# alibaba/nann

Measured on AMD Instinct MI355X. Metric: retrieval QPS @ recall@200 parity, 1M items/128-d, higher is better.
Workload: dtype f16 rows / f32 L2

## Files before the change

nann_amd/csrc/nann_device.h:

```cpp
#pragma once
#include <type_traits>
#include <hip/hip_runtime.h>
#include <hip/hip_fp16.h>
#include <stdint.h>

namespace nann {

constexpr int kNT = 1024;
constexpr int kNW = kNT / 64;
constexpr int kTopkEPT = 16;
constexpr int kMaxK = 1024;
constexpr int kPhaseScratch = 27648;
constexpr int kMaxD = 512;
constexpr int kLdsScoresOff = 10752;
constexpr int kLdsScores = 4096;

enum : int { DT_F16 = 0, DT_BF16 = 1, DT_F32 = 2 };

__device__ __forceinline__ int local_tid() {
  int t = threadIdx.x;
  asm volatile("" : "+v"(t));
  __builtin_assume(t >= 0 && t < 1024);
  return t;
}
// ... 457 lines not shown
  }
  __syncthreads();
  int base = 0;
  for (int c = 0; c < n_chunks; ++c) {
    const bool more = c + 1 < n_chunks;
    if (more) issue(c + 1, first_row(c + 1) + wave, B);
    const int n_c = min(kChunk, G - c * kChunk);
    long long tw = pt.now();
    base = wg_filter_chunk<kLdsBm, NT>(S, n_c, bm, n_items, out, base);
    pt.sub(PH_EX_WALKBUSY, tw);
    if (more) {
      commit(c + 1, B);
      rest(c + 1, B.r0);
    }
    __syncthreads();
  }
  pt.sub(PH_EX_LOOP, tsub);
  const int bad = S->bad;
  __syncthreads();
  return bad ? -1 : base;
}

constexpr uint32_t kVisEmpty = 0xffffffffu;
constexpr int kVisPosBits = 12;
constexpr int kVisStepBits = 6;
template <int NT, int SLOTS>
struct ExpandHashScratch {
  static constexpr int PER = 4096 / NT;
  static constexpr int kMaskBits = 2 * SLOTS;
  static constexpr int kMaskWords = kMaskBits / 32;
  uint32_t rowdelta[kMaxK];
  uint32_t startmask[kMaskWords];
  unsigned short maskprefix[kMaskWords];
  unsigned long long kept[64];
  uint32_t wave_tot[2 * kNW];
  int flags[4];
};

constexpr int kVisTagBits = 14;
constexpr int kVisMinPiece = 512;
constexpr int kVisDirectBits = 32 - kVisPosBits;
template <int SLOTS, bool TAG>
__device__ __forceinline__ void vis_key(int32_t x, int id_bits, uint32_t& h0, uint32_t& hi) {
  static_assert(SLOTS == 16384 || SLOTS == 32768, "14 or 15 hash bits");
  constexpr int HB = SLOTS == 16384 ? 14 : 15;
  if constexpr (!TAG) {
// ... 42 lines not shown
        const uint32_t c = atomicCAS(&vis[h], kVisEmpty, val);
        if (c == kVisEmpty) break;
        if ((c ^ val) < kStepOne) { S->flags[1] = 1; break; }
        if (step_inc && (val & kStepEnd) == kStepEnd) { S->flags[2] = 1; break; }
        h = (h + step) & (SLOTS - 1);
        val += step_inc;
      }
      out[i] = id;
    } else {
      S->flags[0] = 1;
    }
  }
  __syncthreads();
  const int bad = S->flags[0], dup = S->flags[1], far = S->flags[2];
  __syncthreads();
  return bad ? -1 : far ? -2 : dup ? -4 : n;
}

template <int NT, int SLOTS, bool TAG>
__device__ __forceinline__ int wg_expand_hash_impl(const int32_t* frontier, int n_frontier,
                                              const int32_t* __restrict__ values,
                                              const int64_t* __restrict__ row_splits, uint32_t n_items,
                                              uint32_t* vis, int id_bits, int& vis_count, int32_t* out,
                                              unsigned char* scratch, int* gathered, SubTimer pt) {
  using Scratch = ExpandHashScratch<NT, SLOTS>;
  constexpr int PER = Scratch::PER;
  constexpr int NWV = NT / 64;
  static_assert(PER * NWV == 64, "one keep-mask word per lane");
  Scratch* S = reinterpret_cast<Scratch*>(scratch);
  long long tsub = pt.now();
  const int tid = local_tid(), lane = tid & 63;
  const int wave = __builtin_amdgcn_readfirstlane(tid >> 6);
  const uint64_t lt = lanemask_lt(lane);
  const bool list_mode = row_splits == nullptr;
  const int n_rows = list_mode ? 1 : n_frontier;
  if (tid < 4) S->flags[tid] = 0;
  for (int i = tid; i < Scratch::kMaskWords; i += NT) S->startmask[i] = 0u;
  __syncthreads();
  uint32_t total = 0, rows_ne = 0;
  for (int t0 = 0; t0 < n_rows; t0 += NT) {
    const int t = t0 + tid;
    uint32_t len = 0, start = 0;
    if (list_mode) {
      if (t == 0) len = (uint32_t)n_frontier;
    } else if (t < n_frontier) {
      const int32_t node = frontier[t];
      if ((uint32_t)node < n_items) {
        const int64_t s = row_splits[node], e = row_splits[node + 1];
        start = (uint32_t)s;
        len = (uint32_t)(e - s);
      } else {
        S->flags[0] = 1;
      }
    }
    const uint32_t ne = len ? 1u : 0u;
    const uint32_t inc = wave_scan_add(len), inc_ne = wave_scan_add(ne);
    if (lane == 63) { S->wave_tot[wave] = inc; S->wave_tot[kNW + wave] = inc_ne; }
    __syncthreads();
    uint32_t wbase = 0, tot = 0, wbase_ne = 0, tot_ne = 0;
#pragma unroll
    for (int w = 0; w < NWV; ++w) {
      const uint32_t v = S->wave_tot[w], vn = S->wave_tot[kNW + w];
      if (w < wave) { wbase += v; wbase_ne += vn; }
      tot += v; tot_ne += vn;
    }
    const uint32_t my_off = total + wbase + inc - len;
    if (len && my_off < (uint32_t)Scratch::kMaskBits) {
// ... 133 lines not shown
    vis_count += tot;
    if (cut) {
      if (c_next < G) fetch(c_next, min(PL, G - c_next), x);
    } else {
#pragma unroll
      for (int j = 0; j < PER; ++j) x[j] = xn[j];
    }
    c0 = c_next;
    pt.sub(PH_EX_RANK, tw);
  }
  pt.sub(PH_EX_LOOP, tsub);
  if (__ballot(bad) != 0ull && lane == 0) S->flags[0] = 1;
  __syncthreads();
  const int any_bad = S->flags[0];
  __syncthreads();
  return any_bad ? -1 : base;
}

template <int NT, int SLOTS>
__device__ __forceinline__ int wg_expand_hash(const int32_t* frontier, int n_frontier,
                                              const int32_t* __restrict__ values,
                                              const int64_t* __restrict__ row_splits, uint32_t n_items,
                                              uint32_t* vis, int id_bits, int& vis_count, int32_t* out,
                                              unsigned char* scratch, int* gathered, SubTimer pt) {
  if (id_bits <= kVisDirectBits)
    return wg_expand_hash_impl<NT, SLOTS, false>(frontier, n_frontier, values, row_splits, n_items, vis, id_bits,
                                                 vis_count, out, scratch, gathered, pt);
  return wg_expand_hash_impl<NT, SLOTS, true>(frontier, n_frontier, values, row_splits, n_items, vis, id_bits,
                                              vis_count, out, scratch, gathered, pt);
}

template <int DT>
struct RowChunk {
  uint4 a;
  uint4 b;
};

template <int DT>
__device__ __forceinline__ RowChunk<DT> load_chunk(const void* table, size_t row, int d, int sub) {
  RowChunk<DT> r;
  if constexpr (DT == DT_F32) {
    const uint4* p = reinterpret_cast<const uint4*>(static_cast<const float*>(table) + row * d + sub * 8);
    r.a = p[0];
    r.b = p[1];
  } else {
    const uint4* p = reinterpret_cast<const uint4*>(static_cast<const uint16_t*>(table) + row * d + sub * 8);
    r.a = p[0];
    r.b = make_uint4(0, 0, 0, 0);
  }
  return r;
}

// ... 193 lines not shown

template <int KCAP>
struct TopkScratchT {
  unsigned long long sel[KCAP < 512 ? 512 : KCAP];
  union {
    unsigned short prank[kNT];
    struct { uint32_t above[256]; uint32_t cursor[256]; } bins;
  };
  uint32_t misc[4];
  uint32_t wlo[kNW], whi[kNW];
  uint32_t wcnt[kNW];
};
static_assert(kNT * sizeof(unsigned short) == 512 * sizeof(uint32_t), "the bin tables overlay the partial ranks");
typedef TopkScratchT<kMaxK> TopkScratch;
static_assert(sizeof(TopkScratch) <= kLdsScoresOff, "top-k scratch overlaps the LDS scores");
static_assert(kLdsScoresOff + kLdsScores * 4 <= kPhaseScratch, "phase scratch too small");
static_assert(sizeof(ExpandWalkScratch) <= kPhaseScratch, "phase scratch too small");

template <int NS, bool SCL, int NT, int KCAP = kMaxK, bool BIN = false>
__device__ __forceinline__ int wg_topk_impl(const int32_t* ids, const float* scores,
                                            const float* lds_scores, int n, int k, int32_t* out_pos,
                                            int32_t* out_ids, float* out_scores, const int64_t* id_map,
                                            int64_t* out_mapped, unsigned char* scratch, SubTimer pt,
                                            int n_all = 0x7fffffff, uint32_t floor_key = 0u) {
  TopkScratchT<KCAP>* S = reinterpret_cast<TopkScratchT<KCAP>*>(scratch);
  long long tsub = pt.now();
  const int tid = local_tid(), lane = tid & 63, wave = tid >> 6;
  const uint64_t lt = lanemask_lt(lane);
  constexpr bool REG = NS > 0;
  uint32_t key[REG ? NS : 1];
  if constexpr (REG) {
    float raw[NS];
#pragma unroll
    for (int j = 0; j < NS; ++j) {
      const int i = min(j * NT + tid, n - 1);
      raw[j] = SCL ? lds_scores[i] : scores[i];
    }
#pragma unroll
    for (int j = 0; j < NS; ++j) key[j] = (j * NT + tid < n) ? score_key(raw[j]) : 0u;
  }
#define NANN_FOR_KEYS(...)                                                    \
  if constexpr (REG) {                                                        \
    _Pragma("unroll") for (int j = 0; j < NS; ++j) {                          \
      const int i = j * NT + tid;                                             \
      const uint32_t kj = key[j];                                             \
      const bool valid = i < n && (!BIN || i < n_all || kj > floor_key);      \
      __VA_ARGS__                                                             \
// ... 153 lines not shown
      const uint64_t m = __ballot(e);
      if (lane == 0) S->wcnt[wave] = (uint32_t)popc64(m);
      __syncthreads();
      uint32_t wb = 0, tot = 0;
      for (int w = 0; w < NT / 64; ++w) {
        const uint32_t t = S->wcnt[w];
        if (w < wave) wb += t;
        tot += t;
      }
      const uint32_t rank = eq_base + wb + (uint32_t)popc64(m & lt);
      if (e && rank < r) S->sel[c_gt + rank] = ((unsigned long long)kj << 32) | (uint32_t)(~(uint32_t)i);
      eq_base += tot;
      __syncthreads();
    })
  }
#undef NANN_FOR_KEYS
  __syncthreads();
  pt.sub(PH_TK_COLLECT, tsub);
  int K2 = 64;
  while (K2 < k) K2 <<= 1;
  const bool split = K2 <= NT;
  int32_t my_id = 0;
  if (tid < k && ids) my_id = ids[(int)(~(uint32_t)(S->sel[tid] & 0xffffffffull))];
  const bool binned = use_bins && S->misc[3] == 0u;
  if (split && !binned) {
    const int segs = NT / K2;
    const int e = tid & (K2 - 1), seg = tid / K2;
    const int len = (k + segs - 1) / segs;
    const int o0 = seg * len, o1 = min(k, o0 + len);
    int pr = 0;
    if (e < k) {
      const unsigned long long mine = S->sel[e];
      int o = o0;
      for (; o + 8 <= o1; o += 8) {
        unsigned long long v[8];
#pragma unroll
        for (int u = 0; u < 8; ++u) v[u] = S->sel[o + u];
#pragma unroll
        for (int u = 0; u < 8; ++u) pr += (v[u] > mine) ? 1 : 0;
      }
      for (; o < o1; ++o) pr += (S->sel[o] > mine) ? 1 : 0;
    }
    S->prank[tid] = (unsigned short)pr;
    __syncthreads();
  }
  for (int e = tid; e < k; e += NT) {
// ... 15 lines not shown
    } else if (split) {
      for (int sg = 0; sg < NT / K2; ++sg) rank += S->prank[sg * K2 + e];
    } else {
      int o = 0;
      for (; o + 8 <= k; o += 8) {
        unsigned long long v[8];
#pragma unroll
        for (int u = 0; u < 8; ++u) v[u] = S->sel[o + u];
#pragma unroll
        for (int u = 0; u < 8; ++u) rank += (v[u] > mine) ? 1 : 0;
      }
      for (; o < k; ++o) rank += (S->sel[o] > mine) ? 1 : 0;
    }
    const int pos = (int)(~(uint32_t)(mine & 0xffffffffull));
    const int32_t idv = ids ? (e == tid ? my_id : ids[pos]) : pos;
    if (out_pos) out_pos[rank] = pos;
    if (out_ids) out_ids[rank] = idv;
    if (out_scores) {
      const uint32_t kbits = (uint32_t)(mine >> 32);
      const uint32_t u = (kbits & 0x80000000u) ? (kbits & 0x7fffffffu) : ~kbits;
      out_scores[rank] = (u != 0u) ? __uint_as_float(u) : (SCL ? lds_scores[pos] : scores[pos]);
    }
    if (out_mapped) out_mapped[rank] = id_map[idv];
  }
  __syncthreads();
  pt.sub(PH_TK_SORT, tsub);
  return 0;
}

template <int NT = kNT, int KCAP = kMaxK, bool BIN = false>
__device__ __forceinline__ int wg_topk(const int32_t* ids, const float* scores, const float* lds_scores,
                                       int n, int k, int32_t* out_pos, int32_t* out_ids,
                                       float* out_scores, const int64_t* id_map, int64_t* out_mapped,
                                       unsigned char* scratch, SubTimer pt = no_timer()) {
  if (k < 0 || k > KCAP) return 7;
  if (n < k) return 4;
  if (k == 0) return 0;
#define NANN_TOPK_CASE(NS_, SCL_)                                                                   \
  return wg_topk_impl<NS_, SCL_, NT, KCAP, BIN>(ids, scores, lds_scores, n, k, out_pos, out_ids, out_scores, \
                                           id_map, out_mapped, scratch, pt)
  if (lds_scores != nullptr && n <= kLdsScores) {
    if (n <= 1 * NT) NANN_TOPK_CASE(1, true);
    if (n <= 2 * NT) NANN_TOPK_CASE(2, true);
    if (n <= 4 * NT) NANN_TOPK_CASE(4, true);
    if constexpr (8 * NT <= kLdsScores) NANN_TOPK_CASE(8, true);
  }
  if (n <= 1 * NT) NANN_TOPK_CASE(1, false);
  if (n <= 2 * NT) NANN_TOPK_CASE(2, false);
  if (n <= 4 * NT) NANN_TOPK_CASE(4, false);
  if (n <= 8 * NT) NANN_TOPK_CASE(8, false);
  if (n <= kTopkEPT * NT) NANN_TOPK_CASE(kTopkEPT, false);
  NANN_TOPK_CASE(0, false);
#undef NANN_TOPK_CASE
}

template <int NT, int KCAP>
__device__ __forceinline__ int wg_topk_binned(const int32_t* ids, const float* scores, int n, int k, int32_t* out_ids,
                                              float* out_scores, unsigned char* scratch, int n_all = 0x7fffffff,
                                              uint32_t floor_key = 0u) {
  if (k < 0 || k > KCAP) return 7;
  if (n < k) return 4;
  if (k == 0) return 0;
  if (n <= 4 * NT) return wg_topk_impl<4, false, NT, KCAP, true>(ids, scores, nullptr, n, k, nullptr, out_ids, out_scores, nullptr, nullptr, scratch, no_timer(), n_all, floor_key);
// ... 6 lines not shown
```

nann_amd/csrc/nann_hip.hip:

```cpp
#include "nann_eval.h"
#include "nann_attn.h"
#include "nann_order_kernels.h"
#include "nann_scan.h"
#include "host/nann_graphdef_text.h"
#include "host/nann_blaze_options.h"
#include "host/nann_npy.h"
#include "host/nann_projcache.h"

#include <algorithm>
#include <atomic>
#include <cmath>
#include <cstddef>
#include <cstdio>
#include <cstdlib>
#include <cstring>
#include <fstream>
#include <limits>
#include <memory>
#include <mutex>
#include <string>
#include <vector>

#include <sys/stat.h>

// ... 603 lines not shown
    if (hipMemGetInfo(free_b, &total) == hipSuccess) return true;
    (void)hipGetLastError();
    return false;
  }
  static bool event_create(Event* e) {
    if (hipEventCreateWithFlags(e, hipEventDisableTiming) == hipSuccess) return true;
    (void)hipGetLastError();
    return false;
  }
  static void event_destroy(Event e) { (void)hipEventDestroy(e); }
  static void event_record(Event e, Stream s) { (void)hipEventRecord(e, s); }
  static bool event_done(Event e) { return hipEventQuery(e) != hipErrorNotReady; }
  static void event_wait(Event e) { (void)hipEventSynchronize(e); }
};
typedef nann::ProjCacheT<HipProjBackend> ProjCache;
typedef nann::ProjTableT<HipProjBackend> ProjTable;
struct SearchOpt {
  int mode;
  int reserve;
  int preproject;
  int mlp_form;
  int small32;
  int order;
};
static std::atomic<int> g_traversal_mode{-1}, g_slot_reserve{-1}, g_preproject{-1};
static const SearchOpt& env_defaults() {
  static const SearchOpt d = [] {
    SearchOpt o{NANN_TRAVERSAL_AUTO, 0, 1, NANN_MLP_FORM_AUTO, 1, 1};
    if (const char* e = std::getenv("NANN_PREPROJECT")) o.preproject = !(e[0] == '0' && e[1] == 0);
    if (const char* e = std::getenv("NANN_SEARCH_SLOT_RESERVE")) o.reserve = std::max(0, std::atoi(e));
    if (const char* e = std::getenv("NANN_MLP_FORM")) o.mlp_form = std::string(e) == "fused" ? NANN_MLP_FORM_FUSED : std::string(e) == "phased" ? NANN_MLP_FORM_PHASED : NANN_MLP_FORM_AUTO;
    if (const char* e = std::getenv("NANN_PHASE_SMALL32")) o.small32 = !(e[0] == '0');
    if (const char* e = std::getenv("NANN_QUERY_ORDER")) o.order = !(e[0] == '0');
    return o;
  }();
  return d;
}
static SearchOpt resolve_options(const nann_search_options* u) {
  SearchOpt o = env_defaults();
  const int gm = g_traversal_mode.load(std::memory_order_relaxed), gr = g_slot_reserve.load(std::memory_order_relaxed),
            gp = g_preproject.load(std::memory_order_relaxed);
  if (gm >= 0) o.mode = gm;
  if (gr >= 0) o.reserve = gr;
  if (gp >= 0) o.preproject = gp;
  if (u) {
    const size_t nb = u->struct_bytes > 0 ? (size_t)u->struct_bytes : sizeof(*u);
    auto has = [&](const int32_t* f) { return (size_t)(reinterpret_cast<const char*>(f) - reinterpret_cast<const char*>(u)) + 4 <= nb; };
    if (has(&u->traversal_mode) && u->traversal_mode >= 0) o.mode = u->traversal_mode;
    if (has(&u->slot_reserve) && u->slot_reserve >= 0) o.reserve = u->slot_reserve;
    if (has(&u->preprojection) && u->preprojection >= 0) o.preproject = u->preprojection != 0;
    if (has(&u->mlp_form) && u->mlp_form >= 0) o.mlp_form = u->mlp_form;
  }
  return o;
}
static int check_options(const nann_search_options* u) {
  if (!u) return NANN_OK;
// ... 1195 lines not shown
                            : kind < 0 ? big_scratch : (size_t)kPhaseScratch;
  const bool bitmap_fits = !res && bm_bytes + bm_scratch + tail <= di.lds_max;
  const int mode = opt.mode;
  const int bm_vis = (bitmap_fits && mode != NANN_TRAVERSAL_HBM_BITMAP) ? VIS_LDS_BITMAP : VIS_HBM_BITMAP;
  const size_t bm_lds = bm_scratch + tail + (bm_vis == VIS_LDS_BITMAP ? bm_bytes : 0);
  const int bm_per_cu = (bm_vis == VIS_LDS_BITMAP || res) ? 1 : 2;
  const int id_bits = std::max(16, bit_length((uint64_t)std::max<int64_t>(ix->desc.n_items, 1)));
  const bool tag_fits = id_bits <= 27;
  const double mean_deg0 = (double)ix->desc.nb_nnz[0] / (double)std::max<int64_t>(ix->desc.n_items, 1);
  const double walk_deg = std::min<double>((double)ix->max_deg[0], 2.75 * mean_deg0);
  const double rows_walked = (double)t[1] + t[2] + t[3];
  const double est_guess = t[1] + 0.45 * walk_deg * rows_walked;
  const double est_visited = ix->probe_valid ? std::min(t[1] + std::min(1.15 * (double)ix->probe_new_per_row_q90, (double)ix->probe_new_per_row_max) * rows_walked,
                                                        t[1] + (double)ix->max_deg[0] * rows_walked)
                                             : est_guess;
  const bool tag_entries = id_bits > 20;
  const double fit16 = !ix->probe_valid ? 11000.0 : tag_entries ? 13000.0 : 15000.0;
  const double fit32 = !ix->probe_valid ? 24000.0 : tag_entries ? 26000.0 : 30500.0;
  const double worst_visited = t[1] + (double)ix->max_deg[0] * ((double)t[1] + t[2] + t[3]);
  const size_t hash16_lds = (size_t)vis_slots(VIS_LDS_HASH) * 4 + hash_phase_scratch<512, 16384>() + tail;
  const size_t hash32_lds = (size_t)vis_slots(VIS_LDS_HASH32) * 4 + hash_phase_scratch<kNT, 32768>() + tail;
  const bool hash_ok = (kind == NANN_SCORER_L2 || kind < 0) && tag_fits && 2 * hash16_lds <= di.lds_max &&
                       hash32_lds <= di.lds_max;
  int hash_vis = -1;
  if (mode == NANN_TRAVERSAL_LDS_HASH) hash_vis = VIS_LDS_HASH;
  else if (mode == NANN_TRAVERSAL_LDS_HASH32) hash_vis = VIS_LDS_HASH32;
  else if (mode == NANN_TRAVERSAL_AUTO && (kind == NANN_SCORER_L2 || kind < 0)) {
    if (worst_visited <= 16320.0 || est_visited <= fit16) hash_vis = VIS_LDS_HASH;
    else if (worst_visited <= 32704.0 || est_visited <= fit32) hash_vis = VIS_LDS_HASH32;
    if (hash_vis == VIS_LDS_HASH && kind == NANN_SCORER_L2 && n_queries <= (int64_t)di.cus) hash_vis = VIS_LDS_HASH32;
  }
  const bool fits16 = worst_visited <= 16320.0 || est_visited <= fit16 || mode == NANN_TRAVERSAL_LDS_HASH;
  const bool own_hash_plan = (kind == kKindAttn || kind == kKindMlpSplit || res) && tag_fits && fits16;
  if ((mode == NANN_TRAVERSAL_LDS_HASH || mode == NANN_TRAVERSAL_LDS_HASH32) && !hash_ok && kind >= 0 &&
      !(own_hash_plan && mode == NANN_TRAVERSAL_LDS_HASH))
    return fail(NANN_ERR_UNSUPPORTED, "hash-set traversal: shards below 2^27 items; the 32K-slot set: L2 scorer only");
  unsigned long long off[9];
  uint32_t gbm_words = bm_vis == VIS_HBM_BITMAP ? ix->bm_words : 0u;
  if (res || kind < 0 || kind == kKindAttn) gbm_words = std::max<uint32_t>(std::max<uint32_t>(gbm_words, ix->bm_words), (uint32_t)vis_slots(kind < 0 ? VIS_LDS_HASH32 : VIS_LDS_HASH));
  p->slot_bytes = slot_layout(p->max_cand, p->max_raw, p->pool_cap, gbm_words, off);
  p->id_bits = id_bits;
  p->fb_vis = bm_vis;
  p->fb_lds_bytes = bm_lds;
  p->fb_slots = (int)std::max<int64_t>(1, std::min<int64_t>(n_queries, (int64_t)di.cus * bm_per_cu));
  if (own_hash_plan && mode != NANN_TRAVERSAL_LDS_BITMAP && mode != NANN_TRAVERSAL_HBM_BITMAP) {
    p->vis = VIS_LDS_HASH;
    p->nt = 512;
    p->lds_bytes = res ? (size_t)kMlpResBytes + hash_phase_scratch<512, 16384>() + tail
                       : (size_t)vis_slots(VIS_LDS_HASH) * 4 + bm_scratch + tail;
    p->slots = (int)std::max<int64_t>(1, std::min<int64_t>(n_queries, (int64_t)di.cus));
  } else if (hash_ok && hash_vis == VIS_LDS_HASH) {
    p->vis = VIS_LDS_HASH;
    p->nt = 512;
    p->lds_bytes = hash16_lds;
    p->slots = (int)std::max<int64_t>(1, std::min<int64_t>(n_queries, (int64_t)di.cus * 2));
  } else if (hash_ok && hash_vis == VIS_LDS_HASH32) {
    p->vis = VIS_LDS_HASH32;
    p->nt = kNT;
    p->lds_bytes = hash32_lds;
    p->slots = (int)std::max<int64_t>(1, std::min<int64_t>(n_queries, (int64_t)di.cus));
  } else {
    p->vis = bm_vis;
    p->nt = kNT;
    p->lds_bytes = bm_lds;
    p->slots = p->fb_slots;
  }
  const bool exact_form = mlp_exact_hint;
  const bool pays = exact_form || n_queries <= 160;
  const bool no_forced_bitmap = mode != NANN_TRAVERSAL_LDS_BITMAP && mode != NANN_TRAVERSAL_HBM_BITMAP;
  const bool want_phased = opt.mlp_form == NANN_MLP_FORM_PHASED || (opt.mlp_form == NANN_MLP_FORM_AUTO && pays);
  p->phased = res && own_hash_plan && no_forced_bitmap && 2 * hash16_lds <= di.lds_max && want_phased;
  p->phase_vis = VIS_LDS_HASH;
  p->phase_per_cu = 2;
  p->phase_lds_bytes = hash16_lds;
  const bool fits32 = worst_visited <= 32704.0 || est_visited <= fit32;
  if (res && !own_hash_plan && tag_fits && fits32 && no_forced_bitmap && mode != NANN_TRAVERSAL_LDS_HASH && hash32_lds <= di.lds_max &&
      opt.mlp_form != NANN_MLP_FORM_FUSED) {
    p->phased = true;
    p->phase_vis = VIS_LDS_HASH32;
    p->phase_per_cu = 1;
    p->phase_lds_bytes = hash32_lds;
    gbm_words = std::max<uint32_t>(gbm_words, (uint32_t)vis_slots(VIS_LDS_HASH32));
    p->slot_bytes = slot_layout(p->max_cand, p->max_raw, p->pool_cap, gbm_words, off);
  }
  if (p->phased && p->phase_vis == VIS_LDS_HASH && opt.small32 && n_queries <= (int64_t)di.cus && tag_fits && hash32_lds <= di.lds_max) {
    p->phase_vis = VIS_LDS_HASH32;
    p->phase_per_cu = 1;
    p->phase_lds_bytes = hash32_lds;
    gbm_words = std::max<uint32_t>(gbm_words, (uint32_t)vis_slots(VIS_LDS_HASH32));
    p->slot_bytes = slot_layout(p->max_cand, p->max_raw, p->pool_cap, gbm_words, off);
  }
  p->phase_slots = (int)std::max<int64_t>(1, std::min<int64_t>(std::min<int64_t>(n_queries, kPhaseChunk), (int64_t)di.cus * p->phase_per_cu));
  p->phase_score_wgs = di.cus;
  p->est_visited = (float)est_visited;
  p->worst_visited = (float)worst_visited;
  if (kind < 0)
    p->slots = (int)std::max<int64_t>(1, std::min<int64_t>(n_queries, std::max<int64_t>((int64_t)di.cus * 2, kPhaseChunk)));
  else if (const int reserve = opt.reserve) {
    const int per_cu = p->vis == VIS_LDS_HASH && p->nt == 512 && !res && kind != kKindAttn && kind != kKindMlpSplit ? 2
                       : p->vis == VIS_HBM_BITMAP && !res ? 2 : 1;
    p->slots = std::max(1, std::min(p->slots, di.cus * per_cu - reserve));
    p->fb_slots = std::max(1, std::min(p->fb_slots, di.cus * bm_per_cu - reserve));
    p->phase_slots = std::max(1, std::min(p->phase_slots, di.cus * p->phase_per_cu - reserve));
    p->phase_score_wgs = std::max(1, di.cus - (reserve + 1) / 2);
  }
  return NANN_OK;
}

int nann_set_search_reserve(int32_t workgroups) {
  if (workgroups < 0) return fail(NANN_ERR_BAD_ARGUMENT, "nann_set_search_reserve: negative");
  g_slot_reserve.store(workgroups, std::memory_order_relaxed);
// ... 131 lines not shown
    return fail(NANN_ERR_CAPACITY, "workspace smaller than nann_search_workspace_bytes()");
  SearchArgs a;
  a.emb = ix->desc.item_embs;
  a.item_ids = ix->desc.item_ids;
  for (int l = 0; l < 2; ++l) { a.nbv[l] = ix->desc.nb_values[l]; a.nbrs[l] = ix->desc.nb_row_splits[l]; }
  a.enter = ix->desc.enter_points;
  a.n_enter = (int)ix->desc.n_enter;
  a.n_items = (uint32_t)ix->desc.n_items;
  a.d = ix->desc.d;
  a.q = q;
  a.n_queries = (int)n_queries;
  for (int i = 0; i < 6; ++i) a.t[i] = level_topn[i];
  a.tq = tq;
  a.ws = static_cast<unsigned char*>(workspace);
  a.slot_bytes = p.slot_bytes;
  a.bm_words = ix->bm_words;
  a.max_cand = p.max_cand; a.max_raw = p.max_raw; a.pool_cap = p.pool_cap;
  a.out_ids = out_item_ids; a.out_scores = out_scores; a.out_index = out_index;
  a.status = status; a.counters = counters;
  a.phase_ticks = reinterpret_cast<long long*>(phase_ticks);
  a.id_bits = p.id_bits;
  a.redo = 0;
  a.phase = 0;
  a.proj = tab ? tab->table : nullptr;
  a.mlp = MlpParams{};
  a.attn = AttnParams{};
  a.kt = kt; a.upad = upad;
  const int dt = ix->desc.emb_dtype;
  const bool hashed = p.vis == VIS_LDS_HASH || p.vis == VIS_LDS_HASH32;
  const unsigned long long slots_end = 256 + p.slot_bytes * (unsigned long long)std::max(p.slots, p.fb_slots) + kPhaseTail;
  const unsigned long long order_off = ((unsigned long long)workspace_bytes - order_ws_bytes(n_queries)) & ~255ull;
  if (opt.order && hashed && !attn && kind == NANN_SCORER_L2 && ix->n_pivots >= 2 && n_queries > p.slots &&
      (unsigned long long)workspace_bytes >= ((slots_end + 255) & ~255ull) + order_ws_bytes(n_queries)) {
    unsigned char* ow = static_cast<unsigned char*>(workspace) + order_off;
    unsigned int* heads = reinterpret_cast<unsigned int*>(ow);
    int32_t* perm = reinterpret_cast<int32_t*>(ow + kOrderSegs * kOrderHeadStride * 4);
    int32_t* key = perm + n_queries;
    rc = launch_order(ix, q, (int)n_queries, key, perm, heads, static_cast<unsigned int*>(workspace), st);
    if (rc) return rc;
    a.perm = perm;
    a.xheads = heads;
  } else {
    HIP_TRY(hipMemsetAsync(workspace, 0, 256, st));
  }
  auto both = [&](auto&& launch_on) -> int {
    int r2 = launch_on(p.vis, p.nt, p.slots, p.lds_bytes);
// ... 953 lines not shown
```

nann_amd/csrc/nann_search.h:

```cpp
#pragma once
#ifndef NANN_REPEAT_SCORE
#define NANN_REPEAT_SCORE 0
#endif
#ifndef NANN_REPEAT_TOPK
#define NANN_REPEAT_TOPK 0
#endif
#include <type_traits>
#include "../../include/nann_hip.h"
#include "nann_device.h"
#include "nann_order.h"
#include "nann_mlp.h"
#include "nann_mlp2.h"
#include "nann_mlp3.h"
#include "nann_mlp5.h"
#include "nann_mlp6.h"
#include "nann_attn_kernels.h"
#include "nann_attn_split.h"
#include "nann_attn_proj.h"

#include <string>

namespace nann {

struct OpResult {
// ... 79 lines not shown
  int d;
  const float* q;
  int n_queries;
  int t[6];
  const int32_t* tq;
  unsigned char* ws;
  unsigned long long slot_bytes;
  uint32_t bm_words;
  int max_cand, max_raw, pool_cap;
  int64_t* out_ids;
  float* out_scores;
  int32_t* out_index;
  int32_t* status;
  int32_t* counters;
  long long* phase_ticks;
  MlpParams mlp;
  const float* proj;
  AttnParams attn;
  const float* kt;
  const float* upad;
  int id_bits;
  int redo;
  int phase;
  const int32_t* perm = nullptr;
  unsigned int* xheads = nullptr;
};

static_assert(PH_COUNT == NANN_NUM_PHASES, "phase list out of sync with include/nann_hip.h");

struct SlotView {
  int32_t* cand_ids;
  float* cand_scores;
  int32_t* raw;
  int32_t* beam_ids;
  float* beam_scores;
  int32_t* pool_ids;
  float* pool_scores;
  uint32_t* gbitmap;
  PhaseState* phase;
};

__host__ __device__ inline unsigned long long slot_layout(int max_cand, int max_raw, int pool_cap,
                                                          uint32_t gbm_words, unsigned long long off[9]) {
  unsigned long long o = 0;
  auto put = [&](int i, unsigned long long bytes) { off[i] = o; o += (bytes + 255ull) & ~255ull; };
  put(0, 4ull * max_cand);
// ... 29 lines not shown
  VIS_LDS_HASH32 = 3
};
constexpr int vis_slots(int vis) { return vis == VIS_LDS_HASH ? 16384 : vis == VIS_LDS_HASH32 ? 32768 : 0; }

template <int NT, int SLOTS>
constexpr int hash_phase_scratch() {
  constexpr int a = (int)sizeof(TopkScratch), b = (int)sizeof(ExpandHashScratch<NT, SLOTS>);
  return ((a > b ? a : b) + 255) & ~255;
}
constexpr int kAttnSplitScratch = (kAttnSlice + kAttnVecFloats) * 4 + kAttnResidentBytes;
constexpr int kAttnScratch = kAttnSplitScratch > kAttnXResFloats * 4 ? kAttnSplitScratch : kAttnXResFloats * 4;
constexpr int kMlpSplitScratch = (int)((sizeof(MlpSplitScratch) + 255) & ~(size_t)255);
static_assert(sizeof(Mlp2Scratch<128>) <= sizeof(MlpSplitScratch), "the second mapping's tile buffers fit the same phase scratch");
template <int VIS, int SC, int NT>
constexpr int phase_scratch() {
  constexpr bool hash = VIS == VIS_LDS_HASH || VIS == VIS_LDS_HASH32;
  constexpr int base = hash ? hash_phase_scratch<NT, vis_slots(VIS) ? vis_slots(VIS) : 16384>() : kPhaseScratch;
  if (is_mlp_res(SC)) return hash ? base : kMlpResBytes;
  if (is_attn(SC) && base < kAttnScratch) return kAttnScratch;
  if (SC == kScorerMlpSplit && base < kMlpSplitScratch) return kMlpSplitScratch;
  return base;
}

template <int LPR, int DT, int VIS, int SC, int NT>
__device__ __forceinline__ int search_one(const SearchArgs& a, int qi, const SlotView& sv, uint32_t* bm,
                                          unsigned char* scratch, float* qv, int32_t* ctr,
                                          long long* ticks) {
  constexpr bool HASH = VIS == VIS_LDS_HASH || VIS == VIS_LDS_HASH32;
  constexpr bool LDSBM = VIS == VIS_LDS_BITMAP;
  constexpr int SLOTS = HASH ? vis_slots(VIS) : 16384;
  const int tid = local_tid();
  const int k5 = a.t[5];
  if constexpr (SC == kScorerMlpPhase) {
    if (a.phase > 0 && sv.phase->status != kPhasePending) return kPhaseSkip;
  }
  int t[6];
#pragma unroll
  for (int i = 0; i < 6; ++i) t[i] = a.tq ? a.tq[(size_t)qi * 6 + i] : a.t[i];
  if (a.tq) {
    bool bad = false;
#pragma unroll
    for (int i = 0; i < 6; ++i) bad |= t[i] < 0 || t[i] > a.t[i];
    if (bad) return NANN_ERR_BAD_ARGUMENT;
  }
  float* lds_scores = (SC == NANN_SCORER_L2 && !HASH) ? reinterpret_cast<float*>(scratch + kLdsScoresOff) : nullptr;
  PhaseTimer timer;
// ... 3 lines not shown

  if constexpr (!is_attn(SC)) {
    if (SC != kScorerMlpPhase || a.phase == 0)
      for (int k = tid; k < a.d; k += NT) qv[k] = a.q[(size_t)qi * a.d + k];
  }
  __syncthreads();
  constexpr int H1T = 8, H2T = 4;
  float mlp_u = 0.0f;
  if constexpr (SC == NANN_SCORER_MLP || SC == kScorerMlpSplit || is_mlp_res(SC)) mlp_u = wg_mlp_query_u<NT>(a.mlp, qv);
  constexpr bool PHASED = SC == kScorerMlpPhase;
  bool resumed = false;
  if constexpr (PHASED) {
    if (a.phase == 0) {
      const float u = wg_mlp_query_u<NT>(a.mlp, qv);
      if (tid < 256) sv.phase->u[tid] = u;
    } else {
      resumed = true;
      if (tid < 3 * NANN_NUM_ROUNDS) ctr[tid] = sv.phase->ctr[tid];
    }
  }

  constexpr bool kTopkBins = SC == NANN_SCORER_L2;
  int vis_count = 0;
  const int E = a.n_enter;
  int nP = 0;
  const int32_t* frontier = nullptr;
  int nB = 0;
  int r_first = 0;
  if constexpr (PHASED) {
    if (resumed) {
      r_first = a.phase - 1;
      nP = sv.phase->nP;
      vis_count = sv.phase->vis_count;
      if constexpr (HASH) {
        if (r_first == 2 || r_first == 3) {
          const uint4* park = reinterpret_cast<const uint4*>(sv.gbitmap);
          for (int i = tid; i < SLOTS / 4; i += NT) reinterpret_cast<uint4*>(bm)[i] = park[i];
        }
      }
      __syncthreads();
    }
  }
  for (int r = r_first; r <= NANN_NUM_ROUNDS; ++r) {
    const int32_t* sc_ids = nullptr;
    float* sc_out = nullptr;
    int sc_n = 0, base_off = 0;
// ... 40 lines not shown
                if (atomicOr(&bm[(uint32_t)id >> 5], bit) & bit) flags[0] = 1;
                dst[i] = id;
              } else {
                flags[1] = 1;
              }
            }
            __syncthreads();
            const int dup = flags[0], oob = flags[1];
            __syncthreads();
            if (oob) return NANN_ERR_INDEX_OUT_OF_RANGE;
            if (!dup) {
              kept = n_in;
            } else {
              wg_zero_words(bm, a.bm_words);
              __syncthreads();
            }
          }
          if (kept == -3)
            kept = wg_expand_walk<LDSBM, NT>(ss == 0 ? nullptr : frontier, n_in, src, rs, a.n_items, bm, dst,
                                             scratch, &gathered, ss == 0 ? no_timer() : pt);
        } else {
          if (ss == 0) {
            kept = wg_mark_hash<NT, SLOTS>(src, n_in, a.n_items, bm, a.id_bits, dst, scratch);
            if (kept == -4) { wg_vis_clear<SLOTS>(bm); __syncthreads(); kept = -3; }
            else if (kept >= 0) vis_count = kept;
          }
          if (kept == -3)
            kept = wg_expand_hash<NT, SLOTS>(ss == 0 ? nullptr : frontier, n_in, src, rs, a.n_items, bm, a.id_bits,
                                             vis_count, dst, scratch, &gathered, ss == 0 ? no_timer() : pt);
        }
        mark(ss == 0 ? PH_WALK : PH_EXPAND);
        if (kept == -2) return NANN_ERR_CAPACITY;
        if (kept < 0) return NANN_ERR_INDEX_OUT_OF_RANGE;
        if (ss == 0) {
          if (r == 1) {
            if (kept != t[0]) return NANN_ERR_BAD_ARGUMENT;
            base_off = kept;
          }
          frontier = sv.beam_ids;
          nB = kept;
        } else {
          nC = kept; G = gathered;
        }
      }
      if (r == 1) {
        for (int i = tid; i < base_off; i += NT) {
          const float v = sv.beam_scores[i];
          sv.cand_scores[i] = v;
          if (lds_scores != nullptr && i < kLdsScores) lds_scores[i] = v;
        }
      }
      if (tid == 0) { ctr[0 * 5 + r] = nB; ctr[1 * 5 + r] = G; ctr[2 * 5 + r] = nC; }
// ... 127 lines not shown
    if (r == 0) {
      tk_ids = a.enter; tk_sc = sv.cand_scores; tk_n = E; tk_k = t[0];
      tk_out_ids = sv.beam_ids; tk_out_sc = sv.beam_scores;
    } else if (r == 1) {
      tk_ids = sv.cand_ids; tk_sc = sv.cand_scores; tk_n = base_off + sc_n; tk_k = t[1];
      tk_out_ids = sv.pool_ids; tk_out_sc = sv.pool_scores;
    } else if (r < NANN_NUM_ROUNDS) {
      tk_ids = sv.cand_ids; tk_sc = sv.cand_scores; tk_n = sc_n; tk_k = t[r];
      tk_out_ids = sv.pool_ids + nP; tk_out_sc = sv.pool_scores + nP;
    } else {
      tk_ids = sv.pool_ids; tk_sc = sv.pool_scores; tk_n = nP; tk_k = t[5];
      tk_out_ids = a.out_index ? a.out_index + (size_t)qi * k5 : nullptr;
      tk_out_sc = a.out_scores ? a.out_scores + (size_t)qi * k5 : nullptr;
      tk_map = a.item_ids; tk_out_map = a.out_ids + (size_t)qi * k5;
    }
    mark(PH_OTHER);
#if NANN_REPEAT_TOPK
    for (int rep = 0; rep < NANN_REPEAT_TOPK; ++rep) {
      (void)wg_topk<NT, kMaxK, kTopkBins>(tk_ids, tk_sc, (r < NANN_NUM_ROUNDS) ? lds_scores : nullptr, tk_n, tk_k,
                        nullptr, tk_out_ids, tk_out_sc, tk_map, tk_out_map, scratch, pt);
      __syncthreads();
    }
#endif
    const int st = wg_topk<NT, kMaxK, kTopkBins>(tk_ids, tk_sc, (r < NANN_NUM_ROUNDS) ? lds_scores : nullptr, tk_n, tk_k,
                               nullptr, tk_out_ids, tk_out_sc, tk_map, tk_out_map, scratch, pt);
    mark(PH_TOPK);
    if (st) return st;
    if (r == 1) {
      nP = t[1];
    } else if (r >= 2 && r < NANN_NUM_ROUNDS) {
      frontier = sv.pool_ids + nP;
      nB = t[r];
      nP += nB;
    }
  }
  mark(PH_OTHER);
  return NANN_OK;
}

struct WsHeader {
  unsigned int queue;
  unsigned int pad0[15];
  unsigned int redo_queue;
  unsigned int pad1[15];
  unsigned int n_redo;
  unsigned int pad2a;
  unsigned long long refined[NANN_NUM_ROUNDS];
  unsigned int pad2[4];
  unsigned int pqueue[8];
};
// ... 98 lines not shown
      a.counters[(size_t)qi * 3 * NANN_NUM_ROUNDS + threadIdx.x] = s_ctr[threadIdx.x];
    if (a.phase_ticks && threadIdx.x < NANN_NUM_PHASES)
      a.phase_ticks[(size_t)qi * NANN_NUM_PHASES + threadIdx.x] = s_ticks[threadIdx.x];
  }
}

struct SearchPlan {
  int max_cand, max_raw, pool_cap;
  int vis;
  int id_bits;
  size_t lds_bytes;
  unsigned long long slot_bytes;
  int slots;
  int nt;
  int fb_vis;
  size_t fb_lds_bytes;
  int fb_slots;
  bool phased;
  size_t phase_lds_bytes;
  int phase_slots;
  int phase_vis, phase_per_cu;
  int phase_score_wgs;
  float est_visited, worst_visited;
};

template <int LPR, int DT, int VIS, int SC, int NT>
inline int launch_search_as(int slots, size_t lds_bytes, const SearchArgs& a, hipStream_t st) {
  auto kern = k_search<LPR, DT, VIS, SC, NT>;
  if (lds_bytes > 48 * 1024)
    NANN_HIP_TRY(hipFuncSetAttribute(reinterpret_cast<const void*>(kern),
                                     hipFuncAttributeMaxDynamicSharedMemorySize, (int)lds_bytes));
  hipLaunchKernelGGL(kern, dim3(slots), dim3(NT), lds_bytes, st, a);
  NANN_HIP_TRY(hipGetLastError());
  return NANN_OK;
}

template <int LPR, int DT, int SC, int NT>
inline int launch_search_bitmap(int vis, int slots, size_t lds_bytes, const SearchArgs& a, hipStream_t st) {
  if (vis == VIS_LDS_BITMAP) return launch_search_as<LPR, DT, VIS_LDS_BITMAP, SC, NT>(slots, lds_bytes, a, st);
  return launch_search_as<LPR, DT, VIS_HBM_BITMAP, SC, NT>(slots, lds_bytes, a, st);
}

int launch_search_l2_f16(int lpr, int vis, int nt, int slots, size_t lds_bytes, const SearchArgs& a, hipStream_t st);
int launch_search_l2_bf16(int lpr, int vis, int nt, int slots, size_t lds_bytes, const SearchArgs& a, hipStream_t st);
int launch_search_l2_f32(int lpr, int vis, int nt, int slots, size_t lds_bytes, const SearchArgs& a, hipStream_t st);
int launch_search_mlp_d64(int dt, int split, int vis, int slots, size_t lds_bytes, const SearchArgs& a, hipStream_t st);
// ... 25 lines not shown
```

Baseline: 2.864 million.

## Hand off neighbor row ranges from top-k to next round's hash expand

```diff
diff --git a/nann_amd/csrc/nann_device.h b/nann_amd/csrc/nann_device.h
--- a/nann_amd/csrc/nann_device.h
+++ b/nann_amd/csrc/nann_device.h
@@ -503,6 +503,7 @@
 }
 
 constexpr uint32_t kVisEmpty = 0xffffffffu;
+constexpr uint32_t kHandoffBadId = 0xffffffffu;
 constexpr int kVisPosBits = 12;
 constexpr int kVisStepBits = 6;
 template <int NT, int SLOTS>
@@ -591,7 +592,8 @@
                                               const int32_t* __restrict__ values,
                                               const int64_t* __restrict__ row_splits, uint32_t n_items,
                                               uint32_t* vis, int id_bits, int& vis_count, int32_t* out,
-                                              unsigned char* scratch, int* gathered, SubTimer pt) {
+                                              unsigned char* scratch, int* gathered, SubTimer pt,
+                                              const uint2* ho = nullptr) {
   using Scratch = ExpandHashScratch<NT, SLOTS>;
   constexpr int PER = Scratch::PER;
   constexpr int NWV = NT / 64;
@@ -612,6 +614,12 @@
     uint32_t len = 0, start = 0;
     if (list_mode) {
       if (t == 0) len = (uint32_t)n_frontier;
+    } else if (ho != nullptr) {
+      if (t < n_frontier) {
+        const uint2 rg = ho[t];
+        if (rg.y != kHandoffBadId) { start = rg.x; len = rg.y; }
+        else S->flags[0] = 1;
+      }
     } else if (t < n_frontier) {
       const int32_t node = frontier[t];
       if ((uint32_t)node < n_items) {
@@ -791,12 +799,13 @@
                                               const int32_t* __restrict__ values,
                                               const int64_t* __restrict__ row_splits, uint32_t n_items,
                                               uint32_t* vis, int id_bits, int& vis_count, int32_t* out,
-                                              unsigned char* scratch, int* gathered, SubTimer pt) {
+                                              unsigned char* scratch, int* gathered, SubTimer pt,
+                                              const uint2* ho = nullptr) {
   if (id_bits <= kVisDirectBits)
     return wg_expand_hash_impl<NT, SLOTS, false>(frontier, n_frontier, values, row_splits, n_items, vis, id_bits,
-                                                 vis_count, out, scratch, gathered, pt);
+                                                 vis_count, out, scratch, gathered, pt, ho);
   return wg_expand_hash_impl<NT, SLOTS, true>(frontier, n_frontier, values, row_splits, n_items, vis, id_bits,
-                                              vis_count, out, scratch, gathered, pt);
+                                              vis_count, out, scratch, gathered, pt, ho);
 }
 
 template <int DT>
@@ -1036,7 +1045,9 @@
                                             const float* lds_scores, int n, int k, int32_t* out_pos,
                                             int32_t* out_ids, float* out_scores, const int64_t* id_map,
                                             int64_t* out_mapped, unsigned char* scratch, SubTimer pt,
-                                            int n_all = 0x7fffffff, uint32_t floor_key = 0u) {
+                                            int n_all = 0x7fffffff, uint32_t floor_key = 0u,
+                                            const int64_t* __restrict__ ho_splits = nullptr, uint32_t ho_items = 0u,
+                                            uint2* ho = nullptr) {
   TopkScratchT<KCAP>* S = reinterpret_cast<TopkScratchT<KCAP>*>(scratch);
   long long tsub = pt.now();
   const int tid = local_tid(), lane = tid & 63, wave = tid >> 6;
@@ -1236,6 +1247,16 @@
   const bool split = K2 <= NT;
   int32_t my_id = 0;
   if (tid < k && ids) my_id = ids[(int)(~(uint32_t)(S->sel[tid] & 0xffffffffull))];
+  auto row_range = [&](int32_t id) {
+    uint2 rg = make_uint2(0u, kHandoffBadId);
+    if ((uint32_t)id < ho_items) {
+      const int64_t s = ho_splits[id], e = ho_splits[id + 1];
+      rg = make_uint2((uint32_t)s, (uint32_t)(e - s));
+    }
+    return rg;
+  };
+  uint2 my_rg = make_uint2(0u, 0u);
+  if (ho_splits != nullptr && ids != nullptr && tid < k) my_rg = row_range(my_id);
   const bool binned = use_bins && S->misc[3] == 0u;
   if (split && !binned) {
     const int segs = NT / K2;
@@ -1297,6 +1318,7 @@
       out_scores[rank] = (u != 0u) ? __uint_as_float(u) : (SCL ? lds_scores[pos] : scores[pos]);
     }
     if (out_mapped) out_mapped[rank] = id_map[idv];
+    if (ho_splits != nullptr) ho[rank] = (e == tid && ids) ? my_rg : row_range(idv);
   }
   __syncthreads();
   pt.sub(PH_TK_SORT, tsub);
@@ -1307,13 +1329,14 @@
 __device__ __forceinline__ int wg_topk(const int32_t* ids, const float* scores, const float* lds_scores,
                                        int n, int k, int32_t* out_pos, int32_t* out_ids,
                                        float* out_scores, const int64_t* id_map, int64_t* out_mapped,
-                                       unsigned char* scratch, SubTimer pt = no_timer()) {
+                                       unsigned char* scratch, SubTimer pt = no_timer(),
+                                       const int64_t* ho_splits = nullptr, uint32_t ho_items = 0u, uint2* ho = nullptr) {
   if (k < 0 || k > KCAP) return 7;
   if (n < k) return 4;
   if (k == 0) return 0;
 #define NANN_TOPK_CASE(NS_, SCL_)                                                                   \
   return wg_topk_impl<NS_, SCL_, NT, KCAP, BIN>(ids, scores, lds_scores, n, k, out_pos, out_ids, out_scores, \
-                                           id_map, out_mapped, scratch, pt)
+                                           id_map, out_mapped, scratch, pt, 0x7fffffff, 0u, ho_splits, ho_items, ho)
   if (lds_scores != nullptr && n <= kLdsScores) {
     if (n <= 1 * NT) NANN_TOPK_CASE(1, true);
     if (n <= 2 * NT) NANN_TOPK_CASE(2, true);
diff --git a/nann_amd/csrc/nann_hip.hip b/nann_amd/csrc/nann_hip.hip
--- a/nann_amd/csrc/nann_hip.hip
+++ b/nann_amd/csrc/nann_hip.hip
@@ -649,16 +649,18 @@
   int mlp_form;
   int small32;
   int order;
+  int handoff;
 };
 static std::atomic<int> g_traversal_mode{-1}, g_slot_reserve{-1}, g_preproject{-1};
 static const SearchOpt& env_defaults() {
   static const SearchOpt d = [] {
-    SearchOpt o{NANN_TRAVERSAL_AUTO, 0, 1, NANN_MLP_FORM_AUTO, 1, 1};
+    SearchOpt o{NANN_TRAVERSAL_AUTO, 0, 1, NANN_MLP_FORM_AUTO, 1, 1, 1};
     if (const char* e = std::getenv("NANN_PREPROJECT")) o.preproject = !(e[0] == '0' && e[1] == 0);
     if (const char* e = std::getenv("NANN_SEARCH_SLOT_RESERVE")) o.reserve = std::max(0, std::atoi(e));
     if (const char* e = std::getenv("NANN_MLP_FORM")) o.mlp_form = std::string(e) == "fused" ? NANN_MLP_FORM_FUSED : std::string(e) == "phased" ? NANN_MLP_FORM_PHASED : NANN_MLP_FORM_AUTO;
     if (const char* e = std::getenv("NANN_PHASE_SMALL32")) o.small32 = !(e[0] == '0');
     if (const char* e = std::getenv("NANN_QUERY_ORDER")) o.order = !(e[0] == '0');
+    if (const char* e = std::getenv("NANN_EXPAND_HANDOFF")) o.handoff = !(e[0] == '0');
     return o;
   }();
   return d;
@@ -1900,6 +1902,11 @@
   const size_t hash32_lds = (size_t)vis_slots(VIS_LDS_HASH32) * 4 + hash_phase_scratch<kNT, 32768>() + tail;
   const bool hash_ok = (kind == NANN_SCORER_L2 || kind < 0) && tag_fits && 2 * hash16_lds <= di.lds_max &&
                        hash32_lds <= di.lds_max;
+  const int ho_want = opt.handoff ? std::max(std::max(t[0], t[1]), std::max(t[2], t[3])) : 0;
+  const size_t ho_bytes = hash_handoff_bytes(ho_want);
+  const int ho16 = 2 * (hash16_lds + ho_bytes) <= di.lds_max ? ho_want : 0;
+  const int ho32 = hash32_lds + ho_bytes <= di.lds_max ? ho_want : 0;
+  p->ho_cap = p->phase_ho_cap = 0;
   int hash_vis = -1;
   if (mode == NANN_TRAVERSAL_LDS_HASH) hash_vis = VIS_LDS_HASH;
   else if (mode == NANN_TRAVERSAL_LDS_HASH32) hash_vis = VIS_LDS_HASH32;
@@ -1930,12 +1937,14 @@
   } else if (hash_ok && hash_vis == VIS_LDS_HASH) {
     p->vis = VIS_LDS_HASH;
     p->nt = 512;
-    p->lds_bytes = hash16_lds;
+    p->ho_cap = ho16;
+    p->lds_bytes = hash16_lds + hash_handoff_bytes(ho16);
     p->slots = (int)std::max<int64_t>(1, std::min<int64_t>(n_queries, (int64_t)di.cus * 2));
   } else if (hash_ok && hash_vis == VIS_LDS_HASH32) {
     p->vis = VIS_LDS_HASH32;
     p->nt = kNT;
-    p->lds_bytes = hash32_lds;
+    p->ho_cap = ho32;
+    p->lds_bytes = hash32_lds + hash_handoff_bytes(ho32);
     p->slots = (int)std::max<int64_t>(1, std::min<int64_t>(n_queries, (int64_t)di.cus));
   } else {
     p->vis = bm_vis;
@@ -1950,21 +1959,24 @@
   p->phased = res && own_hash_plan && no_forced_bitmap && 2 * hash16_lds <= di.lds_max && want_phased;
   p->phase_vis = VIS_LDS_HASH;
   p->phase_per_cu = 2;
-  p->phase_lds_bytes = hash16_lds;
+  p->phase_ho_cap = ho16;
+  p->phase_lds_bytes = hash16_lds + hash_handoff_bytes(ho16);
   const bool fits32 = worst_visited <= 32704.0 || est_visited <= fit32;
   if (res && !own_hash_plan && tag_fits && fits32 && no_forced_bitmap && mode != NANN_TRAVERSAL_LDS_HASH && hash32_lds <= di.lds_max &&
       opt.mlp_form != NANN_MLP_FORM_FUSED) {
     p->phased = true;
     p->phase_vis = VIS_LDS_HASH32;
     p->phase_per_cu = 1;
-    p->phase_lds_bytes = hash32_lds;
+    p->phase_ho_cap = ho32;
+    p->phase_lds_bytes = hash32_lds + hash_handoff_bytes(ho32);
     gbm_words = std::max<uint32_t>(gbm_words, (uint32_t)vis_slots(VIS_LDS_HASH32));
     p->slot_bytes = slot_layout(p->max_cand, p->max_raw, p->pool_cap, gbm_words, off);
   }
   if (p->phased && p->phase_vis == VIS_LDS_HASH && opt.small32 && n_queries <= (int64_t)di.cus && tag_fits && hash32_lds <= di.lds_max) {
     p->phase_vis = VIS_LDS_HASH32;
     p->phase_per_cu = 1;
-    p->phase_lds_bytes = hash32_lds;
+    p->phase_ho_cap = ho32;
+    p->phase_lds_bytes = hash32_lds + hash_handoff_bytes(ho32);
     gbm_words = std::max<uint32_t>(gbm_words, (uint32_t)vis_slots(VIS_LDS_HASH32));
     p->slot_bytes = slot_layout(p->max_cand, p->max_raw, p->pool_cap, gbm_words, off);
   }
@@ -2142,6 +2154,7 @@
   a.id_bits = p.id_bits;
   a.redo = 0;
   a.phase = 0;
+  a.ho_cap = (mlp_res && p.phased) ? p.phase_ho_cap : p.ho_cap;
   a.proj = tab ? tab->table : nullptr;
   a.mlp = MlpParams{};
   a.attn = AttnParams{};
diff --git a/nann_amd/csrc/nann_search.h b/nann_amd/csrc/nann_search.h
--- a/nann_amd/csrc/nann_search.h
+++ b/nann_amd/csrc/nann_search.h
@@ -125,6 +125,7 @@
   int id_bits;
   int redo;
   int phase;
+  int ho_cap = 0;
   const int32_t* perm = nullptr;
   unsigned int* xheads = nullptr;
 };
@@ -200,6 +201,14 @@
   return base;
 }
 
+constexpr size_t hash_handoff_bytes(int cap) { return ((size_t)cap * sizeof(uint2) + 15) & ~(size_t)15; }
+constexpr int kSearchMiscBytes = 256;
+static_assert(20 * 4 + NANN_NUM_PHASES * 8 <= kSearchMiscBytes, "the misc words of k_search");
+template <int VIS, int SC>
+constexpr bool has_handoff() {
+  return (VIS == VIS_LDS_HASH || VIS == VIS_LDS_HASH32) && (SC == NANN_SCORER_L2 || SC == kScorerMlpPhase);
+}
+
 template <int LPR, int DT, int VIS, int SC, int NT>
 __device__ __forceinline__ int search_one(const SearchArgs& a, int qi, const SlotView& sv, uint32_t* bm,
                                           unsigned char* scratch, float* qv, int32_t* ctr,
@@ -249,6 +258,9 @@
 
   constexpr bool kTopkBins = SC == NANN_SCORER_L2;
   int vis_count = 0;
+  constexpr bool HANDOFF = has_handoff<VIS, SC>();
+  uint2* const ho = reinterpret_cast<uint2*>(reinterpret_cast<unsigned char*>(qv + kMaxD) + kSearchMiscBytes);
+  int ho_n = 0;
   const int E = a.n_enter;
   int nP = 0;
   const int32_t* frontier = nullptr;
@@ -335,12 +347,13 @@
         } else {
           if (ss == 0) {
             kept = wg_mark_hash<NT, SLOTS>(src, n_in, a.n_items, bm, a.id_bits, dst, scratch);
-            if (kept == -4) { wg_vis_clear<SLOTS>(bm); __syncthreads(); kept = -3; }
+            if (kept == -4) { wg_vis_clear<SLOTS>(bm); __syncthreads(); kept = -3; ho_n = 0; }
             else if (kept >= 0) vis_count = kept;
           }
           if (kept == -3)
             kept = wg_expand_hash<NT, SLOTS>(ss == 0 ? nullptr : frontier, n_in, src, rs, a.n_items, bm, a.id_bits,
-                                             vis_count, dst, scratch, &gathered, ss == 0 ? no_timer() : pt);
+                                             vis_count, dst, scratch, &gathered, ss == 0 ? no_timer() : pt,
+                                             (HANDOFF && ss == 1 && ho_n == n_in && n_in > 0) ? ho : nullptr);
         }
         mark(ss == 0 ? PH_WALK : PH_EXPAND);
         if (kept == -2) return NANN_ERR_CAPACITY;
@@ -514,10 +527,15 @@
       __syncthreads();
     }
 #endif
+    const int64_t* ho_rs = nullptr;
+    if constexpr (HANDOFF) {
+      if (r + 1 < NANN_NUM_ROUNDS && tk_k <= a.ho_cap) ho_rs = a.nbrs[r == 0 ? 1 : 0];
+    }
     const int st = wg_topk<NT, kMaxK, kTopkBins>(tk_ids, tk_sc, (r < NANN_NUM_ROUNDS) ? lds_scores : nullptr, tk_n, tk_k,
-                               nullptr, tk_out_ids, tk_out_sc, tk_map, tk_out_map, scratch, pt);
+                               nullptr, tk_out_ids, tk_out_sc, tk_map, tk_out_map, scratch, pt, ho_rs, a.n_items, ho);
     mark(PH_TOPK);
     if (st) return st;
+    ho_n = ho_rs != nullptr ? tk_k : 0;
     if (r == 1) {
       nP = t[1];
     } else if (r >= 2 && r < NANN_NUM_ROUNDS) {
@@ -662,6 +680,7 @@
   int phase_vis, phase_per_cu;
   int phase_score_wgs;
   float est_visited, worst_visited;
+  int ho_cap, phase_ho_cap;
 };
 
 template <int LPR, int DT, int VIS, int SC, int NT>
```

Measured after the change: 2.824 million. 0.986x the previous value.
